# soedinglab/plass

Hardware: AMD Instinct MI355X
Metric: read-overlaps/s per assembly iteration (higher is better)
Workload: dtype u8/u64 (integer hash, byte compare; f32 ratios)

## Files before the change

plass_amd/csrc/assemble.hip:

```cpp
#include "common.hpp"
#include "device_utils.hpp"
#include "posterior_class.hpp"
#include "ref_rules.hpp"
#include "host_util.hpp"
#include <algorithm>
#include <memory>
#include <cstring>

namespace plasship {

struct Item {
    uint32_t target; int32_t score; uint32_t alnLength; float seqId;
    int32_t qStart, qEnd; uint32_t qLen; int32_t dbStart, dbEnd; uint32_t dbLen;
    uint32_t state;
    uint32_t pad;
};

struct AsmArgs {
    SeqView s;
    const uint64_t *qoff; const AlnRec *recs;
    Item *items;
    const uint64_t *arenaOff;
    const uint32_t *leftCap;
    char *arena;
    uint32_t *flags;
    uint32_t *newLen;
    uint64_t *newStart;
    const signed char *mat;
    double lambda, logK, ln2;
    float seqIdThr; uint64_t maxSeqLen; int rescoreMode;
    uint32_t ownLaneMin;
    unsigned long long *stats;
    uint32_t *bigList; uint32_t nBig;
    const uint32_t *bigCount;
    uint32_t *overList; uint32_t *overCount;
    uint32_t queueCap;
    uint32_t *dbgRounds; uint32_t *dbgCycles;
    uint32_t *midList; uint32_t nMid;
    uint32_t *mid32List; uint32_t nMid32;
    uint32_t *smallList; uint32_t nSmall;
    uint32_t *heap;
    const uint32_t *ambKeys; const uint8_t *ambVals; uint32_t ambMask;
    uint32_t *needKeys; uint32_t *needCount; uint32_t needCap;
    uint32_t *redoList; uint32_t *redoCount;
    const uint32_t *queryList; uint32_t nQueryList;
    uint8_t *cmpCache;
    SeqView aa; char *aaArena; const uint64_t *aaArenaOff; const uint32_t *aaLeftCap; uint32_t *aaNewLen; uint64_t *aaNewStart;
};

__device__ __forceinline__ float seqIdThroughText(float f) {
    if (f == 1.0f) return 1.0f;
    const int t = (int) (f * 1000);
    int zeros = 0;
    if ((double) f < 0.10) zeros++;
    if ((double) f < 0.01) zeros++;
    int digits = 1; for (int x = t; x >= 10; x /= 10) digits++;
    double den = 1.0; for (int i = 0; i < digits + zeros; i++) den *= 10.0;
    return (float) ((double) t / den);
}

template <int G> __device__ __forceinline__ void copyBytesG(char *dst, const char *src, unsigned n, int gl) {
    for (unsigned i = 8u * (unsigned) gl; i < n; i += 8u * G) {
        const uint64_t w = loadU64Unaligned(src + i);
// ... 1000 lines not shown
            active = active && nHeap > 0 && !cmp.abort;
        }
        if (valid) {
            if (cmp.abort) a.redoList[atomicAdd(a.redoCount, 1u)] = id;
            else {
                nAln += h; nQRes += seqLen(a.s, id); nResc += qResc; nRescRes += qRescRes;
                for (uint32_t i = 0; i < nUsed; i++) atomicOr(&a.flags[used[i]], 0x80u);
                if (couldExtend) {
                    atomicOr(&a.flags[id], 0x20u); a.newLen[id] = (uint32_t) curLen; a.newStart[id] = aoff + curStart;
                    if (GUIDED) { a.aaNewLen[id] = (uint32_t) aaLen; a.aaNewStart[id] = a.aaArenaOff[id] + aaStart; }
                    nExt++;
                }
            }
        }
    }
    nExt = waveReduceSumU64(nExt); nResc = waveReduceSumU64(nResc); nRescRes = waveReduceSumU64(nRescRes); nAln = waveReduceSumU64(nAln); nQRes = waveReduceSumU64(nQRes);
    if (laneId() == 0) {
        if (nExt) atomicAdd(&a.stats[0], nExt); if (nResc) atomicAdd(&a.stats[1], nResc); if (nRescRes) atomicAdd(&a.stats[2], nRescRes);
        if (nAln) { atomicAdd(&a.stats[3], nAln); atomicAdd(&a.stats[4], nQRes); atomicAdd(&a.stats[5], nRescRes); }
    }
}

template <int G> __device__ __forceinline__ int groupSum(int v) {
    v = rowSum16(v);
#pragma unroll
    for (int o = 16; o < G; o <<= 1) v += __shfl_xor(v, o, G);
    return v;
}
template <int G> __device__ __forceinline__ unsigned long long groupMax(unsigned long long v) {
    v = rowMax16(v);
#pragma unroll
    for (int o = 16; o < G; o <<= 1) { const unsigned long long ok = __shfl_xor(v, o, G); v = (ok > v) ? ok : v; }
    return v;
}
template <int G> __device__ __forceinline__ uint32_t groupRank(uint32_t mine) {
    uint32_t r = rowCountLess16(mine, mine, false);
#pragma unroll
    for (int o = 16; o < G; o += 16) r += rowCountLess16((uint32_t) __shfl_xor((int) mine, o, G), mine, true);
    return r;
}
template <int G> __device__ __forceinline__ unsigned long long groupBallot(bool p) {
    const unsigned long long m = __ballot(p);
    if (G == 64) return m;
    return (m >> ((laneId() / G) * G)) & ((1ULL << G) - 1ULL);
}

template <int G>
__device__ __forceinline__ Rescored rescoreOnDiagonalG(const char *q, unsigned qLen, const char *t, unsigned tLen, int diagonal,
                                                       const signed char *smat, int gl) {
    Rescored r; r.startPos = -1; r.endPos = -1; r.score = 0; r.diagonalLen = 0; r.idExcl = 0;
    const unsigned dist = (unsigned) abs(diagonal);
    unsigned qo, to, len;
    if (diagonal >= 0 && dist < qLen) { qo = dist; to = 0; len = min(tLen, qLen - dist); }
    else if (diagonal < 0 && dist < tLen) { qo = 0; to = dist; len = min(tLen - dist, qLen); }
    else return r;
    r.diagonalLen = len;
    if (len == 0) return r;
    unsigned first, last;
    int s = 0, ids = 0;
    scoreColumnsG<G>(q + qo, t + to, len, smat, gl, first, last, s, ids);
    s = groupSum<G>(s); ids = groupSum<G>(ids);
    r.score = (unsigned) max(s, 0); r.startPos = (int) first; r.endPos = (int) last; r.idExcl = ids;
    return r;
}

template <int G, int WPE>
__global__ __launch_bounds__(256) __attribute__((amdgpu_waves_per_eu(WPE, WPE))) void assembleGroupKernel(AsmArgs a) {
    __shared__ signed char smat[123 * 123 + 7];
    stageScoreTable(smat, a.mat, 256);
    __syncthreads();
    const int gl = threadIdx.x & (G - 1);
    const uint32_t groupsTotal = gridDim.x * (256 / G);
    const uint32_t nWork = (G == 64) ? a.nMid : ((G == 32) ? a.nMid32 : a.nSmall);
    unsigned long long nExt = 0, nResc = 0, nRescRes = 0, nAln = 0, nQRes = 0;
    const uint32_t *workList = (G == 64) ? a.midList : ((G == 32) ? a.mid32List : a.smallList);
    auto loadWord = [&](uint32_t pid) -> uint64_t {
        uint64_t v = 0;
        if (pid != 0xFFFFFFFFu) {
            if (gl == 0) v = a.qoff[pid]; else if (gl == 1) v = a.qoff[pid + 1]; else if (gl == 2) v = a.arenaOff[pid]; else if (gl == 3) v = a.s.offLen[pid]; else if (gl == 4) v = a.leftCap[pid];
        }
        return v;
    };
    uint32_t w = blockIdx.x * (256 / G) + threadIdx.x / G;
    uint32_t idNext = (w < nWork) ? workList[w] : 0xFFFFFFFFu;
    uint64_t wordNext = loadWord(idNext);
    uint32_t idAhead = (w + groupsTotal < nWork) ? workList[w + groupsTotal] : 0xFFFFFFFFu;
    for (; w < nWork; w += groupsTotal) {
        const uint32_t id = idNext;
        const uint64_t h0 = __shfl(wordNext, 0, G), h1 = __shfl(wordNext, 1, G), aoff = __shfl(wordNext, 2, G), qOffLen = __shfl(wordNext, 3, G), qLeftCap = __shfl(wordNext, 4, G);
        idNext = idAhead; wordNext = loadWord(idNext);
        idAhead = (w + 2u * groupsTotal < nWork) ? workList[w + 2u * groupsTotal] : 0xFFFFFFFFu;
        const uint32_t h = (uint32_t) (h1 - h0);
        const char *orig = a.s.data + (qOffLen >> 24);
        unsigned querySeqLen = (unsigned) ((uint32_t) qOffLen & 0xFFFFFFu);
        if (gl == 0) { nAln += h; nQRes += querySeqLen; }
        uint32_t xTarget = 0xFFFFFFFFu, xAlnLen = 0, xQLen = 0, xDbLen = 0, xState = 2, xTLen = 0; uint64_t xTOff = 0;
        int xScore = 0, xQStart = 0, xQEnd = 0, xDbStart = 0, xDbEnd = 0;
        if ((uint32_t) gl < h) {
// ... 109 lines not shown
                const Rescored rs = rescoreOnDiagonalG<G>(qs, querySeqLen, tSeq, tLen, diag, smat, gl);
                nResc += (gl == 0); nRescRes += (gl == 0) ? rs.diagonalLen : 0;
                const int dist = abs(diag);
                int qS, qE, dS, dE;
                if (diag >= 0) { qS = rs.startPos + dist; qE = rs.endPos + dist; dS = rs.startPos; dE = rs.endPos; }
                else { qS = rs.startPos; qE = rs.endPos; dS = rs.startPos + dist; dE = rs.endPos + dist; }
                const float seqId = (float) rs.idExcl / ((float) qE - (float) qS);
                const float spc = (float) rs.score / (float) ((double) rs.diagonalLen + 0.5);
                if (gl == dl) {
                    xQLen = querySeqLen; xDbLen = tLen; xAlnLen = rs.diagonalLen; xScore = (int) (spc * 100);
                    xQStart = qS; xQEnd = qE; xDbStart = dS; xDbEnd = dE;
                    xState = (seqId >= a.seqIdThr) ? 0u : 2u;
                }
            }
            inQueue = (uint32_t) __popcll(groupBallot<G>(xState == 0));
        }
        if (couldExtend) {
            if (gl == 0) { atomicOr(&a.flags[id], 0x20u); a.newLen[id] = (uint32_t) curLen; a.newStart[id] = aoff + curStart; nExt++; }
        }
    }
    nExt = waveReduceSumU64(nExt); nResc = waveReduceSumU64(nResc); nRescRes = waveReduceSumU64(nRescRes); nAln = waveReduceSumU64(nAln); nQRes = waveReduceSumU64(nQRes);
    if (laneId() == 0) {
        if (nExt) atomicAdd(&a.stats[0], nExt); if (nResc) atomicAdd(&a.stats[1], nResc); if (nRescRes) atomicAdd(&a.stats[2], nRescRes);
        const int tier = (G == 16) ? 0 : 1;
        if (nAln) { atomicAdd(&a.stats[3 + 3 * tier], nAln); atomicAdd(&a.stats[4 + 3 * tier], nQRes); atomicAdd(&a.stats[5 + 3 * tier], nRescRes); }
    }
}

__global__ __launch_bounds__(256) void arenaSumKernel(const AlnRec *__restrict__ recs, uint64_t nAln, uint64_t maxSeqLen, unsigned long long *__restrict__ qSum,
                                                      unsigned long long *__restrict__ qSumAa, uint32_t *__restrict__ qCan, int mirror) {
    const int lane = laneId();
    for (uint64_t i = (uint64_t) blockIdx.x * blockDim.x + threadIdx.x; i < nAln; i += (uint64_t) gridDim.x * blockDim.x) {
        const AlnRec r = recs[i];
        const uint32_t id = r.query;
        uint32_t add = 0, addAa = 0; bool can = false;
        if (r.target != id && r.accepted) {
            add = (uint32_t) r.dbLen; addAa = (uint32_t) r.dbLen / 3 + 2;
            int qS = r.qStart, qE = r.qEnd, dS = r.dbStart, dE = r.dbEnd;
            if (mirror && qS > qE) { qS = r.qEnd; qE = r.qStart; dS = r.dbLen - r.dbEnd - 1; dE = r.dbLen - r.dbStart - 1; }
            const bool notBoth = !(dS == 0 && qS == 0);
            const bool rightStart = dS == 0 && (dE != r.dbLen - 1);
            const bool leftStart = qS == 0 && (qE != r.qLen - 1);
            if ((rightStart || leftStart) && notBoth) {
                if (dS == 0) can = (qE == r.qLen - 1) && (r.dbLen - (dE + 1) > 0);
                else if (qS == 0) can = (dE == r.dbLen - 1) && (dS > 0) && ((uint64_t) r.qLen + (uint64_t) dS < maxSeqLen);
            }
        }
        const unsigned long long act = __ballot(1);
        const uint32_t prevId = (uint32_t) __shfl_up((int) id, 1, 64);
        const bool head = lane == 0 || prevId != id;
        const unsigned long long heads = __ballot(head), cans = __ballot(can);
        const int segStart = 63 - __clzll((long long) (heads & (lane == 63 ? ~0ULL : ((2ULL << lane) - 1ULL))));
        const unsigned long long later = lane == 63 ? 0ULL : (heads & ~((2ULL << lane) - 1ULL));
        const int segEnd = (later ? __ffsll((long long) later) - 1 : (int) __popcll(act)) - 1;
#pragma unroll
        for (int d = 1; d < 64; d <<= 1) {
            const uint32_t t = (uint32_t) __shfl_up((int) add, d, 64), ta = (uint32_t) __shfl_up((int) addAa, d, 64);
            if (lane - d >= segStart) { add += t; addAa += ta; }
        }
        if (lane == segEnd) {
            const unsigned long long seg = (segEnd == 63 ? ~0ULL : ((2ULL << segEnd) - 1ULL)) & ~((1ULL << segStart) - 1ULL);
            if (add) atomicAdd(&qSum[id], (unsigned long long) add);
            if (qSumAa && addAa) atomicAdd(&qSumAa[id], (unsigned long long) addAa);
            if (cans & seg) atomicOr(&qCan[id], 1u);
        }
    }
}
__global__ void arenaSizeKernel(SeqView s, const uint64_t *__restrict__ qoff, const unsigned long long *__restrict__ qSum, const unsigned long long *__restrict__ qSumAa,
                                const uint32_t *__restrict__ qCan, uint32_t *__restrict__ leftCap,
                                uint64_t *__restrict__ bytes, int nuclTiers, uint64_t threadBytes,
                                uint64_t *__restrict__ tierA, uint64_t *__restrict__ tierB,
                                const uint32_t *__restrict__ aaLen, uint32_t *__restrict__ aaLeftCap, uint64_t *__restrict__ aaBytes) {
    for (uint32_t id = blockIdx.x * blockDim.x + threadIdx.x; id < s.n; id += gridDim.x * blockDim.x) {
        int tier = -1;
        const uint64_t sum = qSum[id], sumAa = aaBytes ? qSumAa[id] : 0;
        const bool can = qCan[id] != 0;
        leftCap[id] = (uint32_t) std::min<uint64_t>(sum, 0xFFFFFFFFull);
        const uint64_t slice = (sum && can) ? (2 * sum + s.len[id] + 40) : 0;
        bytes[id] = slice;
        if (aaBytes) { aaLeftCap[id] = (uint32_t) std::min<uint64_t>(sumAa, 0xFFFFFFFFull); aaBytes[id] = (sum && can) ? (2 * sumAa + aaLen[id] + 8) : 0; }
        if (sum && can) { const uint64_t h = qoff[id + 1] - qoff[id]; tier = nuclTiers ? ((h <= 256 && slice <= threadBytes) ? 0 : 1) : (h <= 16 ? 0 : (h <= 32 ? 1 : (h <= 64 ? 2 : 3))); }
        tierA[id] = (tier == 0) ? 1ull : ((tier == 1) ? (1ull << 32) : 0ull);
        tierB[id] = (tier == 2) ? 1ull : ((tier == 3) ? (1ull << 32) : 0ull);
    }
}
__global__ void listKernel(uint32_t n, const uint64_t *__restrict__ tierA, const uint64_t *__restrict__ tierB, const uint64_t *__restrict__ posA,
                           const uint64_t *__restrict__ posB, uint32_t *__restrict__ list0, uint32_t *__restrict__ list1, uint32_t *__restrict__ list2,
                           uint32_t *__restrict__ list3) {
    for (uint32_t id = blockIdx.x * blockDim.x + threadIdx.x; id < n; id += gridDim.x * blockDim.x) {
        const uint64_t a = tierA[id], b = tierB[id];
        if (a & 0xFFFFFFFFull) list0[(uint32_t) posA[id]] = id;
        else if (a) list1[(uint32_t) (posA[id] >> 32)] = id;
        else if (b & 0xFFFFFFFFull) list2[(uint32_t) posB[id]] = id;
        else if (b) list3[(uint32_t) (posB[id] >> 32)] = id;
    }
}

constexpr int NW_CLASSES = 16;
__device__ __forceinline__ int nuclWorkClass(uint64_t slice) {
    const int k = 63 - __clzll((long long) (slice | 1ull));
    return NW_CLASSES - 1 - (min(max(k, 9), 9 + NW_CLASSES - 1) - 9);
}
__global__ __launch_bounds__(256) void nuclClassCountKernel(const uint32_t *__restrict__ list, uint32_t n, const uint64_t *__restrict__ bytes, uint32_t *__restrict__ counts) {
    __shared__ uint32_t sCnt[NW_CLASSES];
    if (threadIdx.x < NW_CLASSES) sCnt[threadIdx.x] = 0;
    __syncthreads();
    for (uint32_t i = blockIdx.x * 256 + threadIdx.x; i < n; i += gridDim.x * 256) atomicAdd(&sCnt[nuclWorkClass(bytes[list[i]])], 1u);
    __syncthreads();
    if (threadIdx.x < NW_CLASSES && sCnt[threadIdx.x]) atomicAdd(&counts[threadIdx.x], sCnt[threadIdx.x]);
}
__global__ __launch_bounds__(256) void nuclClassScatterKernel(const uint32_t *__restrict__ list, uint32_t n, const uint64_t *__restrict__ bytes, uint32_t *__restrict__ counts,
                                                              uint32_t *__restrict__ out) {
    __shared__ uint32_t sCnt[NW_CLASSES], sBase[NW_CLASSES];
    for (uint32_t t0 = blockIdx.x * 256; t0 < n; t0 += gridDim.x * 256) {
        if (threadIdx.x < NW_CLASSES) sCnt[threadIdx.x] = 0;
        __syncthreads();
        const uint32_t i = t0 + threadIdx.x;
// ... 355 lines not shown
        (guided && (dAaLens.alloc((M + 1) * 8) != hipSuccess || dAaStart.alloc((M + 2) * 8) != hipSuccess))) { setError("plasship_assemble: out of device memory"); return PLASSHIP_ERR_DEVICE; }
    if (M) {
        const unsigned gridM = (unsigned) std::min<uint64_t>((M + 255) / 256, 8192);
        hipLaunchKernelGGL(extLensKernel, dim3(gridM), dim3(256), 0, st, gMeta.as<ExtMeta>(), M, dLens.as<uint64_t>(), guided ? dAaLens.as<uint64_t>() : (uint64_t *) nullptr);
        if (exclusiveScanU64(st, dLens.as<uint64_t>(), dStart.as<uint64_t>(), M, dTmp2.p, tmp2Bytes) ||
            (guided && exclusiveScanU64(st, dAaLens.as<uint64_t>(), dAaStart.as<uint64_t>(), M, dTmp2.p, tmp2Bytes))) { setError("plasship_assemble: scan failed"); return PLASSHIP_ERR_DEVICE; }
        hipLaunchKernelGGL(extMergeKernel, dim3(gridM), dim3(256), 0, st, gMeta.as<ExtMeta>(), M, dStart.as<uint64_t>(), guided ? dAaStart.as<uint64_t>() : (const uint64_t *) nullptr,
                           dFlags, dNewLen, dNewStart, dAaNewLen, dAaNewStart);
    }
    PH_TRACE(st, "assemble: merged the extended sequences");
    if (!keepTarget) {
        DevBuf gFlags;
        rc = commAllgathervBytes(ctx, dFlags, (uint64_t) N * 4, gFlags, rb); if (rc) return rc;
        if (N) hipLaunchKernelGGL(orFlagsKernel, dim3(gridN), dim3(256), 0, st, gFlags.as<uint32_t>(), N, W, dFlags);
        PH_CHECK(plasship::streamSync(st));
    }
    PH_CHECK(plasship::streamSync(st));
    PH_CHECK(hipGetLastError());
    return PLASSHIP_OK;
}

static bool asmHistOn() { return getenv("PLASSHIP_DEBUG_ASMHIST") != nullptr; }
static int asmHistRecord(hipStream_t st, uint32_t N, const uint64_t *dQoff, const uint32_t *dBigList, uint32_t nBig, const uint32_t *dRounds, const uint32_t *dCycles,
                         uint32_t cap) {
    static int call = 0;
    std::vector<uint32_t> ids(nBig), rounds(N), cycles(N);
    std::vector<uint64_t> qoff((size_t) N + 1);
    if (nBig) PH_COPY_SYNC(st, ids.data(), dBigList, (size_t) nBig * 4, hipMemcpyDeviceToHost);
    PH_COPY_SYNC(st, qoff.data(), dQoff, ((size_t) N + 1) * 8, hipMemcpyDeviceToHost);
    PH_COPY_SYNC(st, rounds.data(), dRounds, (size_t) N * 4, hipMemcpyDeviceToHost);
    PH_COPY_SYNC(st, cycles.data(), dCycles, (size_t) N * 4, hipMemcpyDeviceToHost);
    constexpr int NH = 5, NR = 8;
    uint64_t hq[NH] = {}, hx[NH] = {}, hr[NH] = {}, hc[NH] = {}, hm[NH] = {}, rq[NR] = {}, ct = 0, over = 0, maxH = 0;
    for (uint32_t w = 0; w < nBig; w++) {
        const uint32_t id = ids[w], h = (uint32_t) (qoff[id + 1] - qoff[id]), r = rounds[id] & 0x7FFFFFFFu;
        int b = 0; while (b < NH - 1 && h > (128u << b)) b++;
        int k = 0; if (r) { k = 1; uint32_t e = 1; while (k < NR - 1 && r > e) { e <<= 1; k++; } }
        hq[b]++; hx[b] += rounds[id] >> 31; hr[b] += r; hm[b] = std::max<uint64_t>(hm[b], r); hc[b] += cycles[id]; ct += cycles[id];
        rq[k]++; over += h > cap; maxH = std::max<uint64_t>(maxH, h);
    }
    std::string s = "asmHist call " + std::to_string(call++) + " big queries " + std::to_string(nBig) + " (max h " + std::to_string(maxH) + ", over cap " +
                    std::to_string(cap) + ": " + std::to_string(over) + ") | h bins <=128,<=256,<=512,<=1024,more: queries/extended/mean rounds/max rounds/% ticks";
    for (int b = 0; b < NH; b++) {
        char t[96];
        snprintf(t, sizeof(t), " [%llu %llu %.2f %llu %.1f%%]", (unsigned long long) hq[b], (unsigned long long) hx[b], hq[b] ? (double) hr[b] / hq[b] : 0.0,
                 (unsigned long long) hm[b], ct ? 100.0 * hc[b] / ct : 0.0);
        s += t;
    }
    s += " | rounds 0,1,2,<=4,<=8,<=16,<=32,more:";
    for (int k = 0; k < NR; k++) s += " " + std::to_string(rq[k]);
    fprintf(stderr, "%s\n", s.c_str());
    return PLASSHIP_OK;
}

static int assembleImpl(plasship_ctx *ctx, const plasship_seqdb *db, const plasship_seqdb *aaDb, const plasship_alns *al,
                        const plasship_assemble_params *par, plasship_seqdb **out, plasship_seqdb **outAa, plasship_assemble_stats *stats) {
    const bool guided = aaDb != nullptr;
    const bool nucl = db->dbtype == PLASSHIP_DBTYPE_NUCLEOTIDES;
    if (!nucl && db->dbtype != PLASSHIP_DBTYPE_AMINO_ACIDS) { setError("plasship_assemble: the sequence DB is neither amino acids nor nucleotides"); return PLASSHIP_ERR_ARG; }
    if (par->rescore_mode != 3) { setError("plasship_assemble: only --rescore-mode 3"); return PLASSHIP_ERR_UNSUPPORTED; }
    if (al->nQueries != db->n) { setError("plasship_assemble: alignment list does not belong to the DB"); return PLASSHIP_ERR_ARG; }
    PH_ENTER(ctx);
    hipStream_t st = ctx->stream;
    const uint32_t N = (uint32_t) db->n;
    if (nucl) { const int rcS = finishSelfAlns(ctx, al); if (rcS) return rcS; }
    const uint64_t nLines = al->nSlots;
    DevBuf dLeftCap, dBytes, dArenaOff, dTmp, dItems, dFlags, dNewLen, dNewStart, dMat, dStats, dArena;
    const size_t tmpBytes = exclusiveScanTmpBytes((size_t) N + 2);
    if (dLeftCap.alloc(((size_t) N + 1) * 4) != hipSuccess || dBytes.alloc(((size_t) N + 1) * 8) != hipSuccess || dArenaOff.alloc(((size_t) N + 2) * 8) != hipSuccess ||
        dTmp.alloc(tmpBytes) != hipSuccess || dItems.alloc(std::max<uint64_t>(nLines, 1) * sizeof(Item)) != hipSuccess || dFlags.alloc(((size_t) N + 1) * 4) != hipSuccess ||
        dNewLen.alloc(((size_t) N + 1) * 4) != hipSuccess || dNewStart.alloc(((size_t) N + 1) * 8) != hipSuccess || dMat.alloc(123 * 123) != hipSuccess || dStats.alloc(128) != hipSuccess) {
        setError("plasship_assemble: out of device memory"); return PLASSHIP_ERR_DEVICE;
    }
    PH_CHECK(hipMemsetAsync(dFlags.p, 0, ((size_t) N + 1) * 4, st));
    PH_CHECK(hipMemsetAsync(dNewLen.p, 0, ((size_t) N + 1) * 4, st));
    PH_CHECK(hipMemsetAsync(dStats.p, 0, 128, st));
    PH_CHECK(hipMemcpyAsync(dMat.p, asciiSubMat(nucl), 123 * 123, hipMemcpyHostToDevice, st));
    { const int rcOL = ensureOffLen(ctx, db); if (rcOL) return rcOL; }
    const SeqView sv = db->view();
    PH_CHECK(hipEventRecord(ctx->ev[0], st));
    DevBuf dBigList, dMidList, dMid32List, dSmallList, dTierA, dTierB, dPosA, dPosB, dAaLeftCap, dAaBytes, dAaArenaOff, dAaArena, dAaNewLen, dAaNewStart;
    if (guided && (dAaLeftCap.alloc(((size_t) N + 1) * 4) != hipSuccess || dAaBytes.alloc(((size_t) N + 1) * 8) != hipSuccess || dAaArenaOff.alloc(((size_t) N + 2) * 8) != hipSuccess ||
                   dAaNewLen.alloc(((size_t) N + 1) * 4) != hipSuccess || dAaNewStart.alloc(((size_t) N + 1) * 8) != hipSuccess)) { setError("plasship_assemble: out of device memory"); return PLASSHIP_ERR_DEVICE; }
    if (guided) PH_CHECK(hipMemsetAsync(dAaNewLen.p, 0, ((size_t) N + 1) * 4, st));
    if (dBigList.alloc(((size_t) N + 1) * 4) != hipSuccess || dMidList.alloc(((size_t) N + 1) * 4) != hipSuccess || dMid32List.alloc(((size_t) N + 1) * 4) != hipSuccess ||
        dSmallList.alloc(((size_t) N + 1) * 4) != hipSuccess || dTierA.alloc(((size_t) N + 1) * 8) != hipSuccess || dTierB.alloc(((size_t) N + 1) * 8) != hipSuccess ||
        dPosA.alloc(((size_t) N + 2) * 8) != hipSuccess || dPosB.alloc(((size_t) N + 2) * 8) != hipSuccess) { setError("plasship_assemble: out of device memory"); return PLASSHIP_ERR_DEVICE; }
    DevBuf dQSum, dQSumAa, dQCan;
    if (dQSum.alloc(((size_t) N + 1) * 8) != hipSuccess || dQCan.alloc(((size_t) N + 1) * 4) != hipSuccess || (guided && dQSumAa.alloc(((size_t) N + 1) * 8) != hipSuccess)) { setError("plasship_assemble: out of device memory"); return PLASSHIP_ERR_DEVICE; }
    PH_CHECK(hipMemsetAsync(dQSum.p, 0, ((size_t) N + 1) * 8, st));
    PH_CHECK(hipMemsetAsync(dQCan.p, 0, ((size_t) N + 1) * 4, st));
    if (guided) PH_CHECK(hipMemsetAsync(dQSumAa.p, 0, ((size_t) N + 1) * 8, st));
    if (nLines) hipLaunchKernelGGL(arenaSumKernel, dim3((unsigned) std::min<uint64_t>((nLines + 255) / 256, (uint64_t) ctx->numCU * 32)), dim3(256), 0, st, al->d_recs.as<AlnRec>(), (uint64_t) nLines,
                                       (uint64_t) par->max_seq_len, dQSum.as<unsigned long long>(), guided ? dQSumAa.as<unsigned long long>() : (unsigned long long *) nullptr, dQCan.as<uint32_t>(),
                                       (nucl && !guided) ? 1 : 0);
    if (N) hipLaunchKernelGGL(arenaSizeKernel, dim3(std::min<uint32_t>((N + 255) / 256, 8192)), dim3(256), 0, st, sv, al->d_qoff.as<uint64_t>(), (const unsigned long long *) dQSum.as<unsigned long long>(),
                              (const unsigned long long *) dQSumAa.as<unsigned long long>(), (const uint32_t *) dQCan.as<uint32_t>(), dLeftCap.as<uint32_t>(), dBytes.as<uint64_t>(), nucl ? 1 : 0, (uint64_t) 1 << 30,
                              dTierA.as<uint64_t>(), dTierB.as<uint64_t>(),
                              guided ? aaDb->d_len.as<uint32_t>() : (const uint32_t *) nullptr, dAaLeftCap.as<uint32_t>(), guided ? dAaBytes.as<uint64_t>() : (uint64_t *) nullptr);
    if (guided && exclusiveScanU64(st, dAaBytes.as<uint64_t>(), dAaArenaOff.as<uint64_t>(), N, dTmp.p, tmpBytes)) { setError("plasship_assemble: scan failed"); return PLASSHIP_ERR_DEVICE; }
    if (exclusiveScanU64(st, dTierA.as<uint64_t>(), dPosA.as<uint64_t>(), N, dTmp.p, tmpBytes) || exclusiveScanU64(st, dTierB.as<uint64_t>(), dPosB.as<uint64_t>(), N, dTmp.p, tmpBytes)) {
        setError("plasship_assemble: scan failed"); return PLASSHIP_ERR_DEVICE;
    }
    if (N) hipLaunchKernelGGL(listKernel, dim3(std::min<uint32_t>((N + 255) / 256, 8192)), dim3(256), 0, st, N, dTierA.as<uint64_t>(), dTierB.as<uint64_t>(), dPosA.as<uint64_t>(), dPosB.as<uint64_t>(),
                              dSmallList.as<uint32_t>(), dMid32List.as<uint32_t>(), dMidList.as<uint32_t>(), dBigList.as<uint32_t>());
    if (exclusiveScanU64(st, dBytes.as<uint64_t>(), dArenaOff.as<uint64_t>(), N, dTmp.p, tmpBytes)) { setError("plasship_assemble: scan failed"); return PLASSHIP_ERR_DEVICE; }
    uint64_t arenaBytes = 0, aaArenaBytes = 0;
    uint64_t totA = 0, totB = 0;
    if (guided) PH_CHECK(hipMemcpyAsync(&aaArenaBytes, dAaArenaOff.as<uint64_t>() + N, 8, hipMemcpyDeviceToHost, st));
    PH_CHECK(hipMemcpyAsync(&arenaBytes, dArenaOff.as<uint64_t>() + N, 8, hipMemcpyDeviceToHost, st));
    PH_CHECK(hipMemcpyAsync(&totA, dPosA.as<uint64_t>() + N, 8, hipMemcpyDeviceToHost, st));
    PH_CHECK(hipMemcpyAsync(&totB, dPosB.as<uint64_t>() + N, 8, hipMemcpyDeviceToHost, st));
    PH_CHECK(plasship::streamSync(st));
    const uint32_t cnts[4] = {(uint32_t) totA, (uint32_t) (totA >> 32), (uint32_t) totB, (uint32_t) (totB >> 32)};
    if (dArena.alloc(arenaBytes + 64) != hipSuccess || (guided && dAaArena.alloc(aaArenaBytes + 64) != hipSuccess)) {
        size_t fr = 0, tt = 0; (void) hipMemGetInfo(&fr, &tt);
        setError("plasship_assemble: out of device memory for the extension arena (" + std::to_string(arenaBytes) + " bytes; device free " + std::to_string(fr) + " of " + std::to_string(tt) + ")"); return PLASSHIP_ERR_DEVICE;
    }
    HostEvaluer ev(nucl, db->residues);
    AsmArgs a; memset(&a, 0, sizeof(a));
    a.s = sv; a.qoff = al->d_qoff.as<uint64_t>(); a.recs = al->d_recs.as<AlnRec>(); a.items = dItems.as<Item>(); a.arenaOff = dArenaOff.as<uint64_t>();
    a.leftCap = dLeftCap.as<uint32_t>(); a.arena = dArena.as<char>(); a.flags = dFlags.as<uint32_t>(); a.newLen = dNewLen.as<uint32_t>(); a.newStart = dNewStart.as<uint64_t>();
    a.mat = dMat.as<signed char>(); a.lambda = ev.g[0]; a.logK = ev.logK; a.ln2 = ev.ln2; a.seqIdThr = par->seq_id_thr; a.maxSeqLen = par->max_seq_len; a.rescoreMode = par->rescore_mode;
    a.ownLaneMin = 6;
    a.stats = dStats.as<unsigned long long>();
    a.smallList = dSmallList.as<uint32_t>(); a.nSmall = cnts[0];
    a.mid32List = dMid32List.as<uint32_t>(); a.nMid32 = cnts[1];
    a.midList = dMidList.as<uint32_t>(); a.nMid = cnts[2];
    a.bigList = dBigList.as<uint32_t>(); a.nBig = cnts[3];
    if (!nucl && a.nBig) { const int rcS = finishSelfAlns(ctx, al, dBigList.as<uint32_t>(), a.nBig); if (rcS) return rcS; }
    std::unique_ptr<plasship_seqdb> aaPacked;
    if (guided && !aaDb->contiguous) {
        const int rcP = packedCopyOf(ctx, aaDb, aaPacked); if (rcP) return rcP;
    }
    if (guided) {
        a.aa = (aaPacked ? aaPacked.get() : aaDb)->view(); a.aaArena = dAaArena.as<char>(); a.aaArenaOff = dAaArenaOff.as<uint64_t>(); a.aaLeftCap = dAaLeftCap.as<uint32_t>();
        a.aaNewLen = dAaNewLen.as<uint32_t>(); a.aaNewStart = dAaNewStart.as<uint64_t>();
    }
    DevBuf dHeap, dNeed, dRedo[2], dCnt;
    if (nucl) {
        const uint32_t needCap = 1u << 16;
        if (dHeap.alloc(std::max<uint64_t>(nLines, 1) * 12) != hipSuccess || dNeed.alloc((size_t) needCap * 16) != hipSuccess || dRedo[0].alloc(((size_t) N + 1) * 4) != hipSuccess ||
            dRedo[1].alloc(((size_t) N + 1) * 4) != hipSuccess || dCnt.alloc(8) != hipSuccess) { setError("plasship_assemble: out of device memory"); return PLASSHIP_ERR_DEVICE; }
        a.heap = dHeap.as<uint32_t>();
        if (!ctx->d_cmpCache.p) {
            const size_t cb = (size_t) CMP_LEN * CMP_MM * CMP_LEN * CMP_MM;
            if (ctx->d_cmpCache.alloc(cb) != hipSuccess) { setError("plasship_assemble: out of device memory"); return PLASSHIP_ERR_DEVICE; }
            PH_CHECK(hipMemsetAsync(ctx->d_cmpCache.p, 0, cb, st));
        }
// ... 26 lines not shown
                    if (guided) hipLaunchKernelGGL(assembleNuclThreadKernel<true>, dim3(grid), dim3(NT_BLOCK), 0, st, a);
                    else hipLaunchKernelGGL(assembleNuclThreadKernel<false>, dim3(grid), dim3(NT_BLOCK), 0, st, a);
                }
                launchWave(dMid32List.as<uint32_t>(), cnts[1]);
            } else launchWave(dRedo[(pass + 1) & 1].as<uint32_t>(), nWork);
            uint32_t cnt[2] = {0, 0};
            PH_CHECK(hipMemcpyAsync(cnt, dCnt.p, 8, hipMemcpyDeviceToHost, st));
            PH_CHECK(plasship::streamSync(st));
            PH_CHECK(hipGetLastError());
            nWork = cnt[1];
            if (nWork == 0) break;
            const uint32_t nNeed = std::min(cnt[0], needCap);
            if (nNeed == 0) { setError("plasship_assemble: queries aborted without a missing comparator tuple"); return PLASSHIP_ERR_DEVICE; }
            std::vector<uint32_t> need((size_t) nNeed * 4);
            PH_COPY_SYNC(ctx->stream, need.data(), dNeed.p, need.size() * 4, hipMemcpyDeviceToHost);
            const int rc = ambTableInsert(ctx, need.data(), nNeed);
            if (rc != PLASSHIP_OK) return rc;
        }
        PH_CHECK(hipEventRecord(ctx->ev[3], st));
        for (int e = 4; e <= 7; e++) PH_CHECK(hipEventRecord(ctx->ev[e], st));
    } else {
    const dim3 g16(std::min<uint32_t>((a.nSmall + 15) / 16, (uint32_t) ctx->numCU * 5u)), g64(std::min<uint32_t>((a.nMid + 3) / 4, (uint32_t) ctx->numCU * 4u));
    PH_CHECK(hipEventRecord(ctx->ev[2], st));
    if (a.nSmall) hipLaunchKernelGGL((assembleGroupKernel<16, 5>), g16, dim3(256), 0, st, a);
    PH_CHECK(hipEventRecord(ctx->ev[3], st));
    PH_CHECK(hipEventRecord(ctx->ev[4], st));
    if (a.nMid32) hipLaunchKernelGGL((assembleGroupKernel<32, 5>), dim3(std::min<uint32_t>((a.nMid32 + 7) / 8, (uint32_t) ctx->numCU * 5u)), dim3(256), 0, st, a);
    if (a.nMid) hipLaunchKernelGGL((assembleGroupKernel<64, 4>), g64, dim3(256), 0, st, a);
    PH_CHECK(hipEventRecord(ctx->ev[5], st));
    PH_CHECK(hipEventRecord(ctx->ev[6], st));
    DevBuf dDbgRounds, dDbgCycles;
    const bool hist = asmHistOn() && a.nBig;
    if (hist) {
        if (dDbgRounds.alloc(((size_t) N + 1) * 4) != hipSuccess || dDbgCycles.alloc(((size_t) N + 1) * 4) != hipSuccess) { setError("plasship_assemble: out of device memory"); return PLASSHIP_ERR_DEVICE; }
        PH_CHECK(hipMemsetAsync(dDbgRounds.p, 0, ((size_t) N + 1) * 4, st));
        PH_CHECK(hipMemsetAsync(dDbgCycles.p, 0, ((size_t) N + 1) * 4, st));
        a.dbgRounds = dDbgRounds.as<uint32_t>(); a.dbgCycles = dDbgCycles.as<uint32_t>();
    }
    const bool onChip = tuneInt("ASMQ", 1) != 2;
    const uint32_t qCap = (uint32_t) std::max(0, std::min(tuneInt("ASMQ_CAP", (int) ASMQ_CAP), (int) ASMQ_CAP));
    const dim3 gBig(std::min<uint32_t>((a.nBig + 3) / 4, (uint32_t) ctx->numCU * 4u));
    DevBuf dOverList[2], dOverCount;
    if (a.nBig && onChip) {
        if (dOverList[0].alloc(((size_t) a.nBig + 1) * 4) != hipSuccess || dOverList[1].alloc(((size_t) a.nBig + 1) * 4) != hipSuccess || dOverCount.alloc(8) != hipSuccess) {
            setError("plasship_assemble: out of device memory"); return PLASSHIP_ERR_DEVICE;
        }
        PH_CHECK(hipMemsetAsync(dOverCount.p, 0, 8, st));
        AsmArgs q1 = a; q1.overList = dOverList[0].as<uint32_t>(); q1.overCount = dOverCount.as<uint32_t>(); q1.queueCap = qCap;
        hipLaunchKernelGGL((assembleQueueKernel<ASMQ_CAP1, 4>), dim3(std::min<uint32_t>((a.nBig + 3) / 4, (uint32_t) ctx->numCU * 4u)), dim3(256), 0, st, q1);
        AsmArgs q2 = q1; q2.bigList = dOverList[0].as<uint32_t>(); q2.bigCount = dOverCount.as<uint32_t>(); q2.overList = dOverList[1].as<uint32_t>(); q2.overCount = dOverCount.as<uint32_t>() + 1;
        hipLaunchKernelGGL((assembleQueueKernel<ASMQ_CAP, 2>), dim3(std::min<uint32_t>((a.nBig + 3) / 4, (uint32_t) ctx->numCU * 2u)), dim3(256), 0, st, q2);
        AsmArgs o = a; o.bigList = dOverList[1].as<uint32_t>(); o.bigCount = dOverCount.as<uint32_t>() + 1;
        hipLaunchKernelGGL(assembleBigKernel, gBig, dim3(256), 0, st, o);
    } else if (a.nBig) hipLaunchKernelGGL(assembleBigKernel, gBig, dim3(256), 0, st, a);
    PH_CHECK(hipEventRecord(ctx->ev[7], st));
    if (hist) { const int rcH = asmHistRecord(st, N, a.qoff, a.bigList, a.nBig, a.dbgRounds, a.dbgCycles, onChip ? qCap : 64); if (rcH) return rcH; }
    }
    PH_TRACE(st, "assemble: extension kernels");
    plasship_seqdb *o = nullptr, *oAa = nullptr;
    unsigned long long hs[16] = {0};
    DevBuf dGathered, dGatheredAa;
    const char *arenaP = dArena.as<char>(), *aaArenaP = dAaArena.as<char>();
    if (commOf(ctx)) {
        const int rc = mergeExtended(ctx, N, guided, par->keep_target, dFlags.as<uint32_t>(), dNewLen.as<uint32_t>(), dNewStart.as<uint64_t>(), dArena.as<char>(),
                                     dAaNewLen.as<uint32_t>(), dAaNewStart.as<uint64_t>(), dAaArena.as<char>(), dTmp.p, tmpBytes, dGathered, dGatheredAa);
        if (rc != PLASSHIP_OK) return rc;
        arenaP = dGathered.as<char>(); aaArenaP = dGatheredAa.as<char>();
    }
    int rcOut = buildOutputDB(ctx, db, dFlags.as<uint32_t>(), dNewLen.as<uint32_t>(), dNewStart.as<uint64_t>(), arenaP, par->keep_target, dTmp.p, tmpBytes, &o,
                              dStats.p, hs, 128, guided ? (hipEvent_t) nullptr : ctx->ev[1], guided);
    if (rcOut != PLASSHIP_OK) return rcOut;
    std::unique_ptr<plasship_seqdb> holdO(o), holdAa;
    if (guided) {
        rcOut = buildOutputDB(ctx, aaDb, dFlags.as<uint32_t>(), dAaNewLen.as<uint32_t>(), dAaNewStart.as<uint64_t>(), aaArenaP, par->keep_target, dTmp.p, tmpBytes, &oAa,
                              nullptr, nullptr, 0, nullptr, true);
        if (rcOut != PLASSHIP_OK) return rcOut;
        holdAa.reset(oAa);
    }
    if (guided) { PH_CHECK(hipEventRecord(ctx->ev[1], st)); PH_CHECK(plasship::streamSync(st)); }
// ... 37 lines not shown
```

plass_amd/csrc/device_utils.hpp:

```cpp
#pragma once
#include <hip/hip_runtime.h>
#include <cstdint>

namespace plasship {

constexpr int WAVE = 64;

__device__ __forceinline__ int laneId() { return (int) (threadIdx.x & 63); }

template <int CTRL> __device__ __forceinline__ uint32_t dppMov(uint32_t v) {
    return (uint32_t) __builtin_amdgcn_mov_dpp((int) v, CTRL, 0xF, 0xF, true);
}
template <int CTRL> __device__ __forceinline__ unsigned long long dppMov64(unsigned long long v) {
    const uint32_t lo = dppMov<CTRL>((uint32_t) v), hi = dppMov<CTRL>((uint32_t) (v >> 32));
    return ((unsigned long long) hi << 32) | lo;
}
__device__ __forceinline__ int rowSum16(int v) {
    v += (int) dppMov<0xB1>((uint32_t) v); v += (int) dppMov<0x4E>((uint32_t) v);
    v += (int) dppMov<0x141>((uint32_t) v); v += (int) dppMov<0x140>((uint32_t) v);
    return v;
}
__device__ __forceinline__ unsigned long long rowMax16(unsigned long long v) {
    unsigned long long o;
    o = dppMov64<0xB1>(v); v = o > v ? o : v;
    o = dppMov64<0x4E>(v); v = o > v ? o : v;
    o = dppMov64<0x141>(v); v = o > v ? o : v;
    o = dppMov64<0x140>(v); v = o > v ? o : v;
    return v;
}
__device__ __forceinline__ uint32_t rowMin16U32(uint32_t v) {
    uint32_t o;
    o = dppMov<0xB1>(v); v = o < v ? o : v;
    o = dppMov<0x4E>(v); v = o < v ? o : v;
    o = dppMov<0x141>(v); v = o < v ? o : v;
    o = dppMov<0x140>(v); v = o < v ? o : v;
    return v;
}
__device__ __forceinline__ uint32_t rowOr16(uint32_t v) {
    v |= dppMov<0xB1>(v); v |= dppMov<0x4E>(v); v |= dppMov<0x141>(v); v |= dppMov<0x140>(v);
    return v;
}
template <int N> struct RowCountLess {
    static __device__ __forceinline__ uint32_t run(uint32_t other, uint32_t mine) {
        return ((dppMov<0x120 + N>(other) < mine) ? 1u : 0u) + RowCountLess<N - 1>::run(other, mine);
    }
};
template <> struct RowCountLess<0> { static __device__ __forceinline__ uint32_t run(uint32_t, uint32_t) { return 0u; } };
__device__ __forceinline__ uint32_t rowCountLess16(uint32_t other, uint32_t mine, bool includeUnrotated) {
    return RowCountLess<15>::run(other, mine) + ((includeUnrotated && other < mine) ? 1u : 0u);
}

__device__ __forceinline__ int waveReduceSum(int v) {
#pragma unroll
    for (int o = 32; o > 0; o >>= 1) v += __shfl_xor(v, o, 64);
    return v;
}
__device__ __forceinline__ unsigned long long waveReduceSumU64(unsigned long long v) {
#pragma unroll
    for (int o = 32; o > 0; o >>= 1) v += __shfl_xor(v, o, 64);
    return v;
}
__device__ __forceinline__ int waveReduceMax(int v) {
#pragma unroll
    for (int o = 32; o > 0; o >>= 1) v = max(v, __shfl_xor(v, o, 64));
    return v;
}
__device__ __forceinline__ unsigned waveInclusiveScan(unsigned v) {
    const int l = laneId();
#pragma unroll
    for (int o = 1; o < 64; o <<= 1) { unsigned t = __shfl_up(v, o, 64); if (l >= o) v += t; }
    return v;
}
// ... 25 lines not shown
```

Before: 714.5 million.

## Add 8-lane group tier for queries with at most eight alignments

Adds a fifth work tier for protein queries with at most eight alignment records, processed by an 8-lane-group variant of the assemble kernel so each wave handles eight queries instead of four. This adds 8-lane DPP reductions and rank helpers. It also replaces the two 64-bit tier-flag arrays, their two full-length scans and the list kernel with a byte-per-query tier array, a per-tile count kernel, a small scan over tile partials and a tile-local list-building kernel. The aim is to cut idle lanes on tiny queries and reduce tier-bucketing memory traffic, at the cost of an extra kernel launch and more complex packed 12-bit counters.

```diff
diff --git a/plass_amd/csrc/assemble.hip b/plass_amd/csrc/assemble.hip
--- a/plass_amd/csrc/assemble.hip
+++ b/plass_amd/csrc/assemble.hip
@@ -39,6 +39,7 @@
     uint32_t *midList; uint32_t nMid;
     uint32_t *mid32List; uint32_t nMid32;
     uint32_t *smallList; uint32_t nSmall;
+    uint32_t *narrowList; uint32_t nNarrow;
     uint32_t *heap;
     const uint32_t *ambKeys; const uint8_t *ambVals; uint32_t ambMask;
     uint32_t *needKeys; uint32_t *needCount; uint32_t needCap;
@@ -1085,18 +1086,19 @@
 }
 
 template <int G> __device__ __forceinline__ int groupSum(int v) {
-    v = rowSum16(v);
+    v = rowSum<(G < 16 ? G : 16)>(v);
 #pragma unroll
     for (int o = 16; o < G; o <<= 1) v += __shfl_xor(v, o, G);
     return v;
 }
 template <int G> __device__ __forceinline__ unsigned long long groupMax(unsigned long long v) {
-    v = rowMax16(v);
+    v = rowMax<(G < 16 ? G : 16)>(v);
 #pragma unroll
     for (int o = 16; o < G; o <<= 1) { const unsigned long long ok = __shfl_xor(v, o, G); v = (ok > v) ? ok : v; }
     return v;
 }
 template <int G> __device__ __forceinline__ uint32_t groupRank(uint32_t mine) {
+    if (G == 8) return rowCountLess8(mine);
     uint32_t r = rowCountLess16(mine, mine, false);
 #pragma unroll
     for (int o = 16; o < G; o += 16) r += rowCountLess16((uint32_t) __shfl_xor((int) mine, o, G), mine, true);
@@ -1127,6 +1129,7 @@
     return r;
 }
 
+constexpr int ASM8_WPE = 5;
 template <int G, int WPE>
 __global__ __launch_bounds__(256) __attribute__((amdgpu_waves_per_eu(WPE, WPE))) void assembleGroupKernel(AsmArgs a) {
     __shared__ signed char smat[123 * 123 + 7];
@@ -1134,9 +1137,9 @@
     __syncthreads();
     const int gl = threadIdx.x & (G - 1);
     const uint32_t groupsTotal = gridDim.x * (256 / G);
-    const uint32_t nWork = (G == 64) ? a.nMid : ((G == 32) ? a.nMid32 : a.nSmall);
+    const uint32_t nWork = (G == 64) ? a.nMid : ((G == 32) ? a.nMid32 : ((G == 16) ? a.nSmall : a.nNarrow));
     unsigned long long nExt = 0, nResc = 0, nRescRes = 0, nAln = 0, nQRes = 0;
-    const uint32_t *workList = (G == 64) ? a.midList : ((G == 32) ? a.mid32List : a.smallList);
+    const uint32_t *workList = (G == 64) ? a.midList : ((G == 32) ? a.mid32List : ((G == 16) ? a.smallList : a.narrowList));
     auto loadWord = [&](uint32_t pid) -> uint64_t {
         uint64_t v = 0;
         if (pid != 0xFFFFFFFFu) {
@@ -1292,7 +1295,7 @@
     nExt = waveReduceSumU64(nExt); nResc = waveReduceSumU64(nResc); nRescRes = waveReduceSumU64(nRescRes); nAln = waveReduceSumU64(nAln); nQRes = waveReduceSumU64(nQRes);
     if (laneId() == 0) {
         if (nExt) atomicAdd(&a.stats[0], nExt); if (nResc) atomicAdd(&a.stats[1], nResc); if (nRescRes) atomicAdd(&a.stats[2], nRescRes);
-        const int tier = (G == 16) ? 0 : 1;
+        const int tier = (G <= 16) ? 0 : 1;
         if (nAln) { atomicAdd(&a.stats[3 + 3 * tier], nAln); atomicAdd(&a.stats[4 + 3 * tier], nQRes); atomicAdd(&a.stats[5 + 3 * tier], nRescRes); }
     }
 }
@@ -1336,10 +1339,12 @@
         }
     }
 }
+constexpr int N_TIERS = 5;
+constexpr uint8_t TIER_NARROW = 4, TIER_NONE = 0xFF;
 __global__ void arenaSizeKernel(SeqView s, const uint64_t *__restrict__ qoff, const unsigned long long *__restrict__ qSum, const unsigned long long *__restrict__ qSumAa,
                                 const uint32_t *__restrict__ qCan, uint32_t *__restrict__ leftCap,
                                 uint64_t *__restrict__ bytes, int nuclTiers, uint64_t threadBytes,
-                                uint64_t *__restrict__ tierA, uint64_t *__restrict__ tierB,
+                                uint8_t *__restrict__ tierOf,
                                 const uint32_t *__restrict__ aaLen, uint32_t *__restrict__ aaLeftCap, uint64_t *__restrict__ aaBytes) {
     for (uint32_t id = blockIdx.x * blockDim.x + threadIdx.x; id < s.n; id += gridDim.x * blockDim.x) {
         int tier = -1;
@@ -1349,20 +1354,61 @@
         const uint64_t slice = (sum && can) ? (2 * sum + s.len[id] + 40) : 0;
         bytes[id] = slice;
         if (aaBytes) { aaLeftCap[id] = (uint32_t) std::min<uint64_t>(sumAa, 0xFFFFFFFFull); aaBytes[id] = (sum && can) ? (2 * sumAa + aaLen[id] + 8) : 0; }
-        if (sum && can) { const uint64_t h = qoff[id + 1] - qoff[id]; tier = nuclTiers ? ((h <= 256 && slice <= threadBytes) ? 0 : 1) : (h <= 16 ? 0 : (h <= 32 ? 1 : (h <= 64 ? 2 : 3))); }
-        tierA[id] = (tier == 0) ? 1ull : ((tier == 1) ? (1ull << 32) : 0ull);
-        tierB[id] = (tier == 2) ? 1ull : ((tier == 3) ? (1ull << 32) : 0ull);
-    }
-}
-__global__ void listKernel(uint32_t n, const uint64_t *__restrict__ tierA, const uint64_t *__restrict__ tierB, const uint64_t *__restrict__ posA,
-                           const uint64_t *__restrict__ posB, uint32_t *__restrict__ list0, uint32_t *__restrict__ list1, uint32_t *__restrict__ list2,
-                           uint32_t *__restrict__ list3) {
-    for (uint32_t id = blockIdx.x * blockDim.x + threadIdx.x; id < n; id += gridDim.x * blockDim.x) {
-        const uint64_t a = tierA[id], b = tierB[id];
-        if (a & 0xFFFFFFFFull) list0[(uint32_t) posA[id]] = id;
-        else if (a) list1[(uint32_t) (posA[id] >> 32)] = id;
-        else if (b & 0xFFFFFFFFull) list2[(uint32_t) posB[id]] = id;
-        else if (b) list3[(uint32_t) (posB[id] >> 32)] = id;
+        if (sum && can) { const uint64_t h = qoff[id + 1] - qoff[id]; tier = nuclTiers ? ((h <= 256 && slice <= threadBytes) ? 0 : 1) : (h <= 8 ? (int) TIER_NARROW : (h <= 16 ? 0 : (h <= 32 ? 1 : (h <= 64 ? 2 : 3)))); }
+        tierOf[id] = (tier < 0) ? TIER_NONE : (uint8_t) tier;
+    }
+}
+static_assert(SCAN_TILE < (1 << 12) && N_TIERS * 12 <= 64 && SCAN_BLOCK == 256, "tier counters of a tile: 12-bit fields of one 64-bit word");
+__device__ __forceinline__ unsigned long long tierField(uint8_t t) { return (t < N_TIERS) ? (1ull << (12 * t)) : 0ull; }
+__device__ __forceinline__ uint64_t loadTierBytes(const uint8_t *__restrict__ tierOf, uint32_t n, uint64_t base) {
+    static_assert(SCAN_ITEMS == 8, "eight tier bytes per thread");
+    if (base + 8 <= n) return *reinterpret_cast<const uint64_t *>(tierOf + base);
+    uint64_t w = ~0ull;
+    for (int k = 0; k < 8; k++) if (base + k < n) w = (w & ~(0xFFull << (8 * k))) | ((uint64_t) tierOf[base + k] << (8 * k));
+    return w;
+}
+__global__ __launch_bounds__(SCAN_BLOCK) void tierCountKernel(const uint8_t *__restrict__ tierOf, uint32_t n, uint64_t *__restrict__ partial, uint32_t nTiles) {
+    __shared__ unsigned long long wsum[SCAN_BLOCK / WAVE];
+    const uint64_t w = loadTierBytes(tierOf, n, (uint64_t) blockIdx.x * SCAN_TILE + (uint64_t) threadIdx.x * SCAN_ITEMS);
+    unsigned long long s = 0;
+#pragma unroll
+    for (int k = 0; k < 8; k++) s += tierField((uint8_t) (w >> (8 * k)));
+    s = waveReduceSumU64(s);
+    if (laneId() == 0) wsum[threadIdx.x >> 6] = s;
+    __syncthreads();
+    if (threadIdx.x < N_TIERS) {
+        unsigned long long t = 0;
+        for (int j = 0; j < SCAN_BLOCK / WAVE; j++) t += wsum[j];
+        partial[(size_t) threadIdx.x * (nTiles + 1) + blockIdx.x] = (t >> (12 * threadIdx.x)) & 0xFFFull;
+    }
+}
+struct TierLists { uint32_t *list[N_TIERS]; };
+__global__ __launch_bounds__(SCAN_BLOCK) void tierListKernel(const uint8_t *__restrict__ tierOf, uint32_t n, const uint64_t *__restrict__ tileOff, uint32_t nTiles,
+                                                             TierLists lists) {
+    __shared__ unsigned long long wsum[SCAN_BLOCK / WAVE];
+    const uint64_t base = (uint64_t) blockIdx.x * SCAN_TILE + (uint64_t) threadIdx.x * SCAN_ITEMS;
+    const uint64_t w = loadTierBytes(tierOf, n, base);
+    unsigned long long s = 0;
+#pragma unroll
+    for (int k = 0; k < 8; k++) s += tierField((uint8_t) (w >> (8 * k)));
+    const unsigned long long incl = waveInclusiveScanU64(s);
+    const int wv = threadIdx.x >> 6;
+    if (laneId() == 63) wsum[wv] = incl;
+    __syncthreads();
+    unsigned long long run = incl - s;
+#pragma unroll
+    for (int j = 0; j < SCAN_BLOCK / WAVE; j++) if (j < wv) run += wsum[j];
+    if (s == 0) return;
+#pragma unroll
+    for (int k = 0; k < 8; k++) {
+        const uint8_t t = (uint8_t) (w >> (8 * k));
+        if (t < N_TIERS) {
+            const uint64_t *row = tileOff + (size_t) t * (nTiles + 1);
+            const uint32_t pos = (uint32_t) (row[blockIdx.x] - row[0]) + (uint32_t) ((run >> (12 * t)) & 0xFFFull);
+            uint32_t *list = (t == 0) ? lists.list[0] : ((t == 1) ? lists.list[1] : ((t == 2) ? lists.list[2] : ((t == 3) ? lists.list[3] : lists.list[4])));
+            list[pos] = (uint32_t) (base + k);
+            run += 1ull << (12 * t);
+        }
     }
 }
 
@@ -1764,7 +1810,7 @@
 
 static bool asmHistOn() { return getenv("PLASSHIP_DEBUG_ASMHIST") != nullptr; }
 static int asmHistRecord(hipStream_t st, uint32_t N, const uint64_t *dQoff, const uint32_t *dBigList, uint32_t nBig, const uint32_t *dRounds, const uint32_t *dCycles,
-                         uint32_t cap) {
+                         uint32_t cap, const uint32_t *tierQueries) {
     static int call = 0;
     std::vector<uint32_t> ids(nBig), rounds(N), cycles(N);
     std::vector<uint64_t> qoff((size_t) N + 1);
@@ -1791,6 +1837,8 @@
     }
     s += " | rounds 0,1,2,<=4,<=8,<=16,<=32,more:";
     for (int k = 0; k < NR; k++) s += " " + std::to_string(rq[k]);
+    s += " | tier queries <=8,<=16,<=32,<=64,more:";
+    for (int t = 0; t < 5; t++) s += " " + std::to_string(tierQueries[t]);
     fprintf(stderr, "%s\n", s.c_str());
     return PLASSHIP_OK;
 }
@@ -1821,13 +1869,14 @@
     { const int rcOL = ensureOffLen(ctx, db); if (rcOL) return rcOL; }
     const SeqView sv = db->view();
     PH_CHECK(hipEventRecord(ctx->ev[0], st));
-    DevBuf dBigList, dMidList, dMid32List, dSmallList, dTierA, dTierB, dPosA, dPosB, dAaLeftCap, dAaBytes, dAaArenaOff, dAaArena, dAaNewLen, dAaNewStart;
+    const uint32_t nTiles = (uint32_t) (((size_t) N + SCAN_TILE - 1) / SCAN_TILE);
+    DevBuf dBigList, dMidList, dMid32List, dSmallList, dNarrowList, dTierOf, dTierPart, dAaLeftCap, dAaBytes, dAaArenaOff, dAaArena, dAaNewLen, dAaNewStart;
     if (guided && (dAaLeftCap.alloc(((size_t) N + 1) * 4) != hipSuccess || dAaBytes.alloc(((size_t) N + 1) * 8) != hipSuccess || dAaArenaOff.alloc(((size_t) N + 2) * 8) != hipSuccess ||
                    dAaNewLen.alloc(((size_t) N + 1) * 4) != hipSuccess || dAaNewStart.alloc(((size_t) N + 1) * 8) != hipSuccess)) { setError("plasship_assemble: out of device memory"); return PLASSHIP_ERR_DEVICE; }
     if (guided) PH_CHECK(hipMemsetAsync(dAaNewLen.p, 0, ((size_t) N + 1) * 4, st));
     if (dBigList.alloc(((size_t) N + 1) * 4) != hipSuccess || dMidList.alloc(((size_t) N + 1) * 4) != hipSuccess || dMid32List.alloc(((size_t) N + 1) * 4) != hipSuccess ||
-        dSmallList.alloc(((size_t) N + 1) * 4) != hipSuccess || dTierA.alloc(((size_t) N + 1) * 8) != hipSuccess || dTierB.alloc(((size_t) N + 1) * 8) != hipSuccess ||
-        dPosA.alloc(((size_t) N + 2) * 8) != hipSuccess || dPosB.alloc(((size_t) N + 2) * 8) != hipSuccess) { setError("plasship_assemble: out of device memory"); return PLASSHIP_ERR_DEVICE; }
+        dSmallList.alloc(((size_t) N + 1) * 4) != hipSuccess || (!nucl && dNarrowList.alloc(((size_t) N + 1) * 4) != hipSuccess) || dTierOf.alloc((size_t) N + 8) != hipSuccess ||
+        dTierPart.alloc(((size_t) N_TIERS * (nTiles + 1) + 1) * 8) != hipSuccess) { setError("plasship_assemble: out of device memory"); return PLASSHIP_ERR_DEVICE; }
     DevBuf dQSum, dQSumAa, dQCan;
     if (dQSum.alloc(((size_t) N + 1) * 8) != hipSuccess || dQCan.alloc(((size_t) N + 1) * 4) != hipSuccess || (guided && dQSumAa.alloc(((size_t) N + 1) * 8) != hipSuccess)) { setError("plasship_assemble: out of device memory"); return PLASSHIP_ERR_DEVICE; }
     PH_CHECK(hipMemsetAsync(dQSum.p, 0, ((size_t) N + 1) * 8, st));
@@ -1838,23 +1887,27 @@
                                        (nucl && !guided) ? 1 : 0);
     if (N) hipLaunchKernelGGL(arenaSizeKernel, dim3(std::min<uint32_t>((N + 255) / 256, 8192)), dim3(256), 0, st, sv, al->d_qoff.as<uint64_t>(), (const unsigned long long *) dQSum.as<unsigned long long>(),
                               (const unsigned long long *) dQSumAa.as<unsigned long long>(), (const uint32_t *) dQCan.as<uint32_t>(), dLeftCap.as<uint32_t>(), dBytes.as<uint64_t>(), nucl ? 1 : 0, (uint64_t) 1 << 30,
-                              dTierA.as<uint64_t>(), dTierB.as<uint64_t>(),
+                              dTierOf.as<uint8_t>(),
                               guided ? aaDb->d_len.as<uint32_t>() : (const uint32_t *) nullptr, dAaLeftCap.as<uint32_t>(), guided ? dAaBytes.as<uint64_t>() : (uint64_t *) nullptr);
     if (guided && exclusiveScanU64(st, dAaBytes.as<uint64_t>(), dAaArenaOff.as<uint64_t>(), N, dTmp.p, tmpBytes)) { setError("plasship_assemble: scan failed"); return PLASSHIP_ERR_DEVICE; }
-    if (exclusiveScanU64(st, dTierA.as<uint64_t>(), dPosA.as<uint64_t>(), N, dTmp.p, tmpBytes) || exclusiveScanU64(st, dTierB.as<uint64_t>(), dPosB.as<uint64_t>(), N, dTmp.p, tmpBytes)) {
-        setError("plasship_assemble: scan failed"); return PLASSHIP_ERR_DEVICE;
-    }
-    if (N) hipLaunchKernelGGL(listKernel, dim3(std::min<uint32_t>((N + 255) / 256, 8192)), dim3(256), 0, st, N, dTierA.as<uint64_t>(), dTierB.as<uint64_t>(), dPosA.as<uint64_t>(), dPosB.as<uint64_t>(),
-                              dSmallList.as<uint32_t>(), dMid32List.as<uint32_t>(), dMidList.as<uint32_t>(), dBigList.as<uint32_t>());
+    PH_CHECK(hipMemsetAsync(dTierPart.p, 0, ((size_t) N_TIERS * (nTiles + 1) + 1) * 8, st));
+    if (nTiles) hipLaunchKernelGGL(tierCountKernel, dim3(nTiles), dim3(SCAN_BLOCK), 0, st, (const uint8_t *) dTierOf.as<uint8_t>(), N, dTierPart.as<uint64_t>(), nTiles);
+    if (exclusiveScanU64(st, dTierPart.as<uint64_t>(), dTierPart.as<uint64_t>(), (size_t) N_TIERS * (nTiles + 1), dTmp.p, tmpBytes)) { setError("plasship_assemble: scan failed"); return PLASSHIP_ERR_DEVICE; }
+    {
+        TierLists tl;
+        tl.list[0] = dSmallList.as<uint32_t>(); tl.list[1] = dMid32List.as<uint32_t>(); tl.list[2] = dMidList.as<uint32_t>(); tl.list[3] = dBigList.as<uint32_t>();
+        tl.list[TIER_NARROW] = dNarrowList.as<uint32_t>();
+        if (nTiles) hipLaunchKernelGGL(tierListKernel, dim3(nTiles), dim3(SCAN_BLOCK), 0, st, (const uint8_t *) dTierOf.as<uint8_t>(), N, (const uint64_t *) dTierPart.as<uint64_t>(), nTiles, tl);
+    }
     if (exclusiveScanU64(st, dBytes.as<uint64_t>(), dArenaOff.as<uint64_t>(), N, dTmp.p, tmpBytes)) { setError("plasship_assemble: scan failed"); return PLASSHIP_ERR_DEVICE; }
     uint64_t arenaBytes = 0, aaArenaBytes = 0;
-    uint64_t totA = 0, totB = 0;
+    uint64_t rowStart[N_TIERS + 1] = {};
     if (guided) PH_CHECK(hipMemcpyAsync(&aaArenaBytes, dAaArenaOff.as<uint64_t>() + N, 8, hipMemcpyDeviceToHost, st));
     PH_CHECK(hipMemcpyAsync(&arenaBytes, dArenaOff.as<uint64_t>() + N, 8, hipMemcpyDeviceToHost, st));
-    PH_CHECK(hipMemcpyAsync(&totA, dPosA.as<uint64_t>() + N, 8, hipMemcpyDeviceToHost, st));
-    PH_CHECK(hipMemcpyAsync(&totB, dPosB.as<uint64_t>() + N, 8, hipMemcpyDeviceToHost, st));
+    PH_CHECK(hipMemcpy2DAsync(rowStart, 8, dTierPart.p, (size_t) (nTiles + 1) * 8, 8, N_TIERS + 1, hipMemcpyDeviceToHost, st));
     PH_CHECK(plasship::streamSync(st));
-    const uint32_t cnts[4] = {(uint32_t) totA, (uint32_t) (totA >> 32), (uint32_t) totB, (uint32_t) (totB >> 32)};
+    uint32_t cnts[N_TIERS];
+    for (int t = 0; t < N_TIERS; t++) cnts[t] = (uint32_t) (rowStart[t + 1] - rowStart[t]);
     if (dArena.alloc(arenaBytes + 64) != hipSuccess || (guided && dAaArena.alloc(aaArenaBytes + 64) != hipSuccess)) {
         size_t fr = 0, tt = 0; (void) hipMemGetInfo(&fr, &tt);
         setError("plasship_assemble: out of device memory for the extension arena (" + std::to_string(arenaBytes) + " bytes; device free " + std::to_string(fr) + " of " + std::to_string(tt) + ")"); return PLASSHIP_ERR_DEVICE;
@@ -1867,6 +1920,7 @@
     a.ownLaneMin = 6;
     a.stats = dStats.as<unsigned long long>();
     a.smallList = dSmallList.as<uint32_t>(); a.nSmall = cnts[0];
+    a.narrowList = dNarrowList.as<uint32_t>(); a.nNarrow = cnts[TIER_NARROW];
     a.mid32List = dMid32List.as<uint32_t>(); a.nMid32 = cnts[1];
     a.midList = dMidList.as<uint32_t>(); a.nMid = cnts[2];
     a.bigList = dBigList.as<uint32_t>(); a.nBig = cnts[3];
@@ -1939,6 +1993,7 @@
     } else {
     const dim3 g16(std::min<uint32_t>((a.nSmall + 15) / 16, (uint32_t) ctx->numCU * 5u)), g64(std::min<uint32_t>((a.nMid + 3) / 4, (uint32_t) ctx->numCU * 4u));
     PH_CHECK(hipEventRecord(ctx->ev[2], st));
+    if (a.nNarrow) hipLaunchKernelGGL((assembleGroupKernel<8, ASM8_WPE>), dim3(std::min<uint32_t>((a.nNarrow + 31) / 32, (uint32_t) ctx->numCU * ASM8_WPE)), dim3(256), 0, st, a);
     if (a.nSmall) hipLaunchKernelGGL((assembleGroupKernel<16, 5>), g16, dim3(256), 0, st, a);
     PH_CHECK(hipEventRecord(ctx->ev[3], st));
     PH_CHECK(hipEventRecord(ctx->ev[4], st));
@@ -1947,7 +2002,8 @@
     PH_CHECK(hipEventRecord(ctx->ev[5], st));
     PH_CHECK(hipEventRecord(ctx->ev[6], st));
     DevBuf dDbgRounds, dDbgCycles;
-    const bool hist = asmHistOn() && a.nBig;
+    const bool hist = asmHistOn();
+    const uint32_t tierQ[5] = {a.nNarrow, a.nSmall, a.nMid32, a.nMid, a.nBig};
     if (hist) {
         if (dDbgRounds.alloc(((size_t) N + 1) * 4) != hipSuccess || dDbgCycles.alloc(((size_t) N + 1) * 4) != hipSuccess) { setError("plasship_assemble: out of device memory"); return PLASSHIP_ERR_DEVICE; }
         PH_CHECK(hipMemsetAsync(dDbgRounds.p, 0, ((size_t) N + 1) * 4, st));
@@ -1971,7 +2027,7 @@
         hipLaunchKernelGGL(assembleBigKernel, gBig, dim3(256), 0, st, o);
     } else if (a.nBig) hipLaunchKernelGGL(assembleBigKernel, gBig, dim3(256), 0, st, a);
     PH_CHECK(hipEventRecord(ctx->ev[7], st));
-    if (hist) { const int rcH = asmHistRecord(st, N, a.qoff, a.bigList, a.nBig, a.dbgRounds, a.dbgCycles, onChip ? qCap : 64); if (rcH) return rcH; }
+    if (hist) { const int rcH = asmHistRecord(st, N, a.qoff, a.bigList, a.nBig, a.dbgRounds, a.dbgCycles, onChip ? qCap : 64, tierQ); if (rcH) return rcH; }
     }
     PH_TRACE(st, "assemble: extension kernels");
     plasship_seqdb *o = nullptr, *oAa = nullptr;
diff --git a/plass_amd/csrc/device_utils.hpp b/plass_amd/csrc/device_utils.hpp
--- a/plass_amd/csrc/device_utils.hpp
+++ b/plass_amd/csrc/device_utils.hpp
@@ -15,19 +15,24 @@
     const uint32_t lo = dppMov<CTRL>((uint32_t) v), hi = dppMov<CTRL>((uint32_t) (v >> 32));
     return ((unsigned long long) hi << 32) | lo;
 }
-__device__ __forceinline__ int rowSum16(int v) {
+template <int W> __device__ __forceinline__ int rowSum(int v) {
+    static_assert(W == 8 || W == 16, "a row of 16 lanes or half of one");
     v += (int) dppMov<0xB1>((uint32_t) v); v += (int) dppMov<0x4E>((uint32_t) v);
-    v += (int) dppMov<0x141>((uint32_t) v); v += (int) dppMov<0x140>((uint32_t) v);
+    v += (int) dppMov<0x141>((uint32_t) v);
+    if (W == 16) v += (int) dppMov<0x140>((uint32_t) v);
     return v;
 }
-__device__ __forceinline__ unsigned long long rowMax16(unsigned long long v) {
+template <int W> __device__ __forceinline__ unsigned long long rowMax(unsigned long long v) {
+    static_assert(W == 8 || W == 16, "a row of 16 lanes or half of one");
     unsigned long long o;
     o = dppMov64<0xB1>(v); v = o > v ? o : v;
     o = dppMov64<0x4E>(v); v = o > v ? o : v;
     o = dppMov64<0x141>(v); v = o > v ? o : v;
-    o = dppMov64<0x140>(v); v = o > v ? o : v;
+    if (W == 16) { o = dppMov64<0x140>(v); v = o > v ? o : v; }
     return v;
 }
+__device__ __forceinline__ int rowSum16(int v) { return rowSum<16>(v); }
+__device__ __forceinline__ unsigned long long rowMax16(unsigned long long v) { return rowMax<16>(v); }
 __device__ __forceinline__ uint32_t rowMin16U32(uint32_t v) {
     uint32_t o;
     o = dppMov<0xB1>(v); v = o < v ? o : v;
@@ -48,6 +53,12 @@
 template <> struct RowCountLess<0> { static __device__ __forceinline__ uint32_t run(uint32_t, uint32_t) { return 0u; } };
 __device__ __forceinline__ uint32_t rowCountLess16(uint32_t other, uint32_t mine, bool includeUnrotated) {
     return RowCountLess<15>::run(other, mine) + ((includeUnrotated && other < mine) ? 1u : 0u);
+}
+
+__device__ __forceinline__ uint32_t rowCountLess8(uint32_t mine) {
+    const uint32_t far = dppMov<0x141>(mine);
+    return ((dppMov<0x39>(mine) < mine) ? 1u : 0u) + ((dppMov<0x4E>(mine) < mine) ? 1u : 0u) + ((dppMov<0x93>(mine) < mine) ? 1u : 0u) +
+           ((far < mine) ? 1u : 0u) + ((dppMov<0x39>(far) < mine) ? 1u : 0u) + ((dppMov<0x4E>(far) < mine) ? 1u : 0u) + ((dppMov<0x93>(far) < mine) ? 1u : 0u);
 }
 
 __device__ __forceinline__ int waveReduceSum(int v) {
```

Result: faster. 723.7 million, median of 6 (+1.3%).
